# PRBonn/OverlapNet

Measured on AMD Instinct MI355X. Metric: scan-pairs/s (64x900 range images), higher is better.
Workload: dtype f32 (scaled 3-term fp16 split on the fp16 MFMA: 22 significand bits per operand, fp32 accumulate)

## Files before the change

overlapnet_amd/csrc/c3_dense.hip:

```cpp
#include "ovn_internal.h"

typedef _Float16 f16x8 __attribute__((ext_vector_type(8)));
typedef _Float16 f16x4 __attribute__((ext_vector_type(4)));

namespace {

struct ArithF16 {
  typedef _Float16 elem;
  typedef f16x8 v8;
  typedef f16x4 v4;
  static __device__ __forceinline__ f32x4 mfma(v8 a, v8 b, f32x4 c) { return __builtin_amdgcn_mfma_f32_16x16x32_f16(a, b, c, 0, 0, 0); }
};

constexpr int G = OVN_G;
constexpr int OW = OVN_O3_HW;
constexpr int CI = OVN_C2_OUT;
constexpr int CO = OVN_C3_OUT;
constexpr int NBAND = 3;
constexpr int MAX_ROWS = 8;
constexpr int MAX_MT = (MAX_ROWS * OW + 15) / 16;
constexpr int IN_PIX_MAX = (MAX_ROWS + 2) * G;
constexpr int PLANE = IN_PIX_MAX * 8 + 8;
constexpr int NPL = CI / 8;
constexpr size_t LDS_BYTES = 2 * (size_t)NPL * PLANE * sizeof(_Float16) + 64;
constexpr int NW = 8;

__device__ __forceinline__ int band_start(int b) { return b == 0 ? 0 : (b == 1 ? 8 : 15); }
__device__ __forceinline__ int band_rows(int b) { return b == 0 ? 8 : 7; }

constexpr int MT_SPLIT = 6;
template <class A, int NWV, int MSPLIT>
__global__ __launch_bounds__(64 * NWV) void c3_dense_kernel(const float* __restrict__ o2, const typename A::elem* __restrict__ wp,
                                                           const float* __restrict__ b3, const float* __restrict__ wd,
                                                           const unsigned* __restrict__ o2max, float sw3,
                                                           float* __restrict__ partial, float* __restrict__ o3,
                                                           unsigned* __restrict__ arrived, const float* __restrict__ bd,
                                                           float* __restrict__ overlap, float* __restrict__ logit) {
  typedef typename A::elem elem_t;
  typedef typename A::v8 v8_t;
  typedef typename A::v4 v4_t;
  extern __shared__ __attribute__((aligned(16))) unsigned char smem[];
  elem_t* ih = reinterpret_cast<elem_t*>(smem);
  elem_t* il = ih + NPL * PLANE;
  float* red = reinterpret_cast<float*>(il + NPL * PLANE);

  constexpr int HALVES = NW / NWV;
  constexpr int MTW = MSPLIT == 1 ? MAX_MT : MT_SPLIT;
  const int sub = blockIdx.x % (HALVES * MSPLIT);
  const int unit = blockIdx.x / (HALVES * MSPLIT), half = sub % HALVES, mh = sub / HALVES;
  const int mt0 = MT_SPLIT * mh;
  const int pair = unit / NBAND;
  const int band = unit - pair * NBAND;
  const int r0 = band_start(band);
  const int nrows = band_rows(band);
  const int npix = nrows * OW;
  const int nmt = (npix + 15) >> 4;
  const int tid = threadIdx.x;
  const int lane = tid & 63;
  const int wave_l = tid >> 6;
  const int wave = wave_l + NWV * half;
  const int lrow = lane & 15;
  const int g = lane >> 4;

  const elem_t* wsrc = wp + ((size_t)(2 * wave) * 2) * 512 + lane * 8;
  v8_t bq[3][4];
#define C3_LOAD_B(DST, KC)                                                                  \
  {                                                                                         \
    const elem_t* q = wsrc + (size_t)(KC) * (16 * 2 * 512);                                 \
    DST[0] = *reinterpret_cast<const v8_t*>(q);                                           \
    DST[1] = *reinterpret_cast<const v8_t*>(q + 512);                                     \
    DST[2] = *reinterpret_cast<const v8_t*>(q + 1024);                                    \
    DST[3] = *reinterpret_cast<const v8_t*>(q + 1536);                                    \
  }
  C3_LOAD_B(bq[0], 0)
  C3_LOAD_B(bq[1], 1)
  const float s2 = ovn_pow2_scale_for(__uint_as_float(o2max[pair]));
  const float inv = 1.0f / (s2 * sw3);
  {
    const float* src = o2 + ((long long)pair * G + r0) * G * CI;
    const int n4 = (nrows + 2) * G * CI / 4;
    constexpr int PER_THREAD = (MAX_ROWS + 2) * G * CI / 4 / (64 * NWV);
    static_assert(PER_THREAD * 64 * NWV == (MAX_ROWS + 2) * G * CI / 4, "patch does not divide over the threads");
    f32x4 v[PER_THREAD];
#pragma unroll
    for (int k = 0; k < PER_THREAD; ++k) {
      const int i = tid + k * (64 * NWV);
      v[k] = (i < n4) ? *reinterpret_cast<const f32x4*>(src + 4 * i) : (f32x4){0.f, 0.f, 0.f, 0.f};
    }
#pragma unroll
    for (int k = 0; k < PER_THREAD; ++k) {
      const int i = tid + k * (64 * NWV);
      if (i < n4) {
        const int pix = i / (CI / 4);
        const int c = 4 * (i - pix * (CI / 4));
        v4_t h, l;
#pragma unroll
        for (int e = 0; e < 4; ++e) {
          const float x = v[k][e] * s2;
          h[e] = (elem_t)x;
          l[e] = (elem_t)(x - (float)h[e]);
        }
        const int o = (c >> 3) * PLANE + pix * 8 + (c & 7);
        *reinterpret_cast<v4_t*>(ih + o) = h;
        *reinterpret_cast<v4_t*>(il + o) = l;
      }
    }
  }

  int abase[MTW];
#pragma unroll
  for (int mt = 0; mt < MTW; ++mt) {
    int p = 16 * (mt0 + mt) + lrow;
    if (p >= npix) p = npix - 1;
    const int oy = p / OW;
    const int ox = p - oy * OW;
    abase[mt] = g * PLANE + (oy * G + ox) * 8;
  }

  f32x4 acc[MTW][2];
#pragma unroll
  for (int mt = 0; mt < MTW; ++mt) {
    acc[mt][0] = (f32x4){0.f, 0.f, 0.f, 0.f};
    acc[mt][1] = (f32x4){0.f, 0.f, 0.f, 0.f};
  }

#define C3_MFMA2(M0, M1, A0H, A0L, A1H, A1L, SRC)                                                  \
  acc[M0][0] = A::mfma(A0H, SRC[0], acc[M0][0]);          \
  acc[M0][1] = A::mfma(A0H, SRC[2], acc[M0][1]);          \
  acc[M1][0] = A::mfma(A1H, SRC[0], acc[M1][0]);          \
  acc[M1][1] = A::mfma(A1H, SRC[2], acc[M1][1]);          \
  acc[M0][0] = A::mfma(A0L, SRC[0], acc[M0][0]);          \
  acc[M0][1] = A::mfma(A0L, SRC[2], acc[M0][1]);          \
  acc[M1][0] = A::mfma(A1L, SRC[0], acc[M1][0]);          \
  acc[M1][1] = A::mfma(A1L, SRC[2], acc[M1][1]);          \
  acc[M0][0] = A::mfma(A0H, SRC[1], acc[M0][0]);          \
  acc[M0][1] = A::mfma(A0H, SRC[3], acc[M0][1]);          \
  acc[M1][0] = A::mfma(A1H, SRC[1], acc[M1][0]);          \
  acc[M1][1] = A::mfma(A1H, SRC[3], acc[M1][1]);
#define C3_READ_A(BUF, SLOT, MT)                                                            \
  fh[BUF][SLOT] = *reinterpret_cast<const v8_t*>(ih + abase[MT] + toff);                  \
  fl[BUF][SLOT] = *reinterpret_cast<const v8_t*>(il + abase[MT] + toff);
#define C3_STEP(SRC, KC)                                                                    \
  {                                                                                         \
    const int tap = (KC) >> 2;                                                              \
    const int ky = tap / 3;                                                                 \
    const int toff = (ky * G + (tap - 3 * ky)) * 8 + 4 * PLANE * ((KC) & 3);                \
    v8_t fh[2][2], fl[2][2];                                                              \
    C3_READ_A(0, 0, 0)                                                                      \
    C3_READ_A(0, 1, 1)                                                                      \
    _Pragma("unroll") for (int q = 0; q < MTW / 2; ++q) {                                \
      const int cb = q & 1, nb = cb ^ 1;                                                    \
      if (q + 1 < MTW / 2) {                                                             \
        C3_READ_A(nb, 0, 2 * q + 2)                                                         \
        C3_READ_A(nb, 1, 2 * q + 3)                                                         \
      } else if (MTW % 2 == 1 && nmt == MAX_MT) {                                                           \
        C3_READ_A(nb, 0, MTW - 1)                                                        \
      }                                                                                     \
      __builtin_amdgcn_sched_barrier(0);   \
      C3_MFMA2(2 * q, 2 * q + 1, fh[cb][0], fl[cb][0], fh[cb][1], fl[cb][1], SRC)           \
      __builtin_amdgcn_sched_barrier(0);                                                    \
    }                                                                                       \
    if (MTW % 2 == 1 && nmt == MAX_MT) {                               \
      const v8_t ah = fh[(MTW / 2) & 1][0], al = fl[(MTW / 2) & 1][0];              \
      acc[MTW - 1][0] = A::mfma(ah, SRC[0], acc[MTW - 1][0]); \
      acc[MTW - 1][1] = A::mfma(ah, SRC[2], acc[MTW - 1][1]); \
      acc[MTW - 1][0] = A::mfma(al, SRC[0], acc[MTW - 1][0]); \
      acc[MTW - 1][1] = A::mfma(al, SRC[2], acc[MTW - 1][1]); \
      acc[MTW - 1][0] = A::mfma(ah, SRC[1], acc[MTW - 1][0]); \
      acc[MTW - 1][1] = A::mfma(ah, SRC[3], acc[MTW - 1][1]); \
    }                                                                                       \
  }
  __syncthreads();
#pragma unroll 1
  for (int kc = 0; kc < 36; kc += 3) {
    C3_LOAD_B(bq[2], kc + 2)
    C3_STEP(bq[0], kc)
    if (kc + 3 < 36) C3_LOAD_B(bq[0], kc + 3)
    C3_STEP(bq[1], kc + 1)
    if (kc + 4 < 36) C3_LOAD_B(bq[1], kc + 4)
    C3_STEP(bq[2], kc + 2)
  }
#undef C3_LOAD_B
#undef C3_STEP
#undef C3_MFMA2
#undef C3_READ_A

  float s[2] = {0.f, 0.f};
#pragma unroll
  for (int nt = 0; nt < 2; ++nt) {
    const int n = 32 * wave + 16 * nt + lrow;
    const float bv = b3[n];
#pragma unroll
    for (int mt = 0; mt < MTW; ++mt) {
#pragma unroll
      for (int r = 0; r < 4; ++r) {
        const int p = 16 * (mt0 + mt) + 4 * g + r;
        if (p < npix) {
          const float v = fmaxf(fmaf(acc[mt][nt][r], inv, bv), 0.0f);
          const long long fi = (long long)(r0 * OW + p) * CO + n;
          s[(MSPLIT == 1 && mt >= MT_SPLIT) ? 1 : 0] += v * wd[fi];
          if (o3) o3[(long long)pair * OVN_DENSE_IN + fi] = v;
        }
      }
    }
  }
#pragma unroll
  for (int off = 32; off > 0; off >>= 1) {
    s[0] += __shfl_down(s[0], off, 64);
    if (MSPLIT == 1) s[1] += __shfl_down(s[1], off, 64);
  }
  if (lane == 0) {
    red[wave_l] = s[0];
    if (MSPLIT == 1) red[NW + wave_l] = s[1];
  }
  __syncthreads();
  if (tid == 0) {
    float* dst = partial + ((size_t)pair * NBAND + band) * 4;
    if (NWV == NW) {
      dst[0] = (red[0] + red[1]) + (red[2] + red[3]);
      dst[1] = (red[NW + 0] + red[NW + 1]) + (red[NW + 2] + red[NW + 3]);
      dst[2] = (red[4] + red[5]) + (red[6] + red[7]);
      dst[3] = (red[NW + 4] + red[NW + 5]) + (red[NW + 6] + red[NW + 7]);
    } else {
      dst[2 * half + mh] = (red[0] + red[1]) + (red[2] + red[3]);
    }
    if (overlap != nullptr) {
      constexpr unsigned PARTS = NBAND * HALVES * MSPLIT;
      __threadfence();
      const unsigned prev = atomicAdd(arrived + pair, 1u);
      if (prev == PARTS - 1) {
        __threadfence();
        const float* q = partial + (size_t)pair * OVN_DENSE_PARTIALS;
        float z = 0.f;
#pragma unroll
        for (int b = 0; b < NBAND; ++b) {
          const float q0 = __hip_atomic_load(q + 4 * b, __ATOMIC_RELAXED, __HIP_MEMORY_SCOPE_AGENT);
          const float q1 = __hip_atomic_load(q + 4 * b + 1, __ATOMIC_RELAXED, __HIP_MEMORY_SCOPE_AGENT);
          const float q2 = __hip_atomic_load(q + 4 * b + 2, __ATOMIC_RELAXED, __HIP_MEMORY_SCOPE_AGENT);
          const float q3 = __hip_atomic_load(q + 4 * b + 3, __ATOMIC_RELAXED, __HIP_MEMORY_SCOPE_AGENT);
          const float zb = (q0 + q1) + (q2 + q3);
          z = b == 0 ? zb : z + zb;
        }
        z += bd[0];
        if (logit) logit[pair] = z;
        overlap[pair] = 1.0f / (1.0f + expf(-z));
        __hip_atomic_store(arrived + pair, 0u, __ATOMIC_RELAXED, __HIP_MEMORY_SCOPE_AGENT);
      }
    }
  }
}

__global__ __launch_bounds__(256) void dense_finish_kernel(const float* __restrict__ partial, const float* __restrict__ bd, int n,
                                                           float* __restrict__ overlap, float* __restrict__ logit) {
  const int p = blockIdx.x * 256 + threadIdx.x;
  if (p >= n) return;
  const float* q = partial + (size_t)p * OVN_DENSE_PARTIALS;
  float z = 0.f;
#pragma unroll
  for (int b = 0; b < NBAND; ++b) {
    const float zb = (q[4 * b] + q[4 * b + 1]) + (q[4 * b + 2] + q[4 * b + 3]);
    z = b == 0 ? zb : z + zb;
  }
  z += bd[0];
  if (logit) logit[p] = z;
  overlap[p] = 1.0f / (1.0f + expf(-z));
}

}

int ovn_c3_dense_forward(const ovn_ctx* ctx, const float* o2, const unsigned* o2max, int n, float* partial, float* o3,
                         unsigned* arrived, float* overlap, float* logit, hipStream_t stream) {
  OVN_REQUIRE(o2max != nullptr, OVN_ERR_ARG, "ovn_c3_dense_forward: the per-pair maxima of o2 are required");
  OVN_REQUIRE(overlap == nullptr || arrived != nullptr, OVN_ERR_ARG, "ovn_c3_dense_forward: arrival counters missing");
  int rc;
  if (n <= 21) {
    rc = ovn_allow_dynamic_lds(reinterpret_cast<const void*>(c3_dense_kernel<ArithF16, 4, 2>), LDS_BYTES);
    if (rc) return rc;
    hipLaunchKernelGGL((c3_dense_kernel<ArithF16, 4, 2>), dim3(4 * NBAND * n), dim3(64 * 4), LDS_BYTES, stream, o2,
                       reinterpret_cast<const _Float16*>(ctx->c3.wp_h), ctx->c3.bias, ctx->wd, o2max, ctx->c3.sw_h, partial, o3, arrived,
                       ctx->bd, overlap, logit);
  } else {
    rc = ovn_allow_dynamic_lds(reinterpret_cast<const void*>(c3_dense_kernel<ArithF16, NW, 1>), LDS_BYTES);
    if (rc) return rc;
    hipLaunchKernelGGL((c3_dense_kernel<ArithF16, NW, 1>), dim3(NBAND * n), dim3(64 * NW), LDS_BYTES, stream, o2,
                       reinterpret_cast<const _Float16*>(ctx->c3.wp_h), ctx->c3.bias, ctx->wd, o2max, ctx->c3.sw_h, partial, o3,
                       (unsigned*)nullptr, ctx->bd, (float*)nullptr, (float*)nullptr);
    if (overlap != nullptr)
      hipLaunchKernelGGL(dense_finish_kernel, dim3((n + 255) / 256), dim3(256), 0, stream, partial, ctx->bd, n, overlap, logit);
  }
  OVN_HIP_CHECK(hipGetLastError());
  return OVN_OK;
}
```

overlapnet_amd/csrc/ovn_api.hip:

```cpp
#include <stdarg.h>
#include <mutex>
#include <set>
#include <utility>
#include <stdio.h>
#include <stdlib.h>
#include <string.h>

#include <algorithm>
#include "ovn_internal.h"

int ovn_allow_dynamic_lds(const void* kernel, size_t bytes) {
  static std::mutex mu;
  static std::set<std::pair<const void*, int>> done;
  int dev = 0;
  OVN_HIP_CHECK(hipGetDevice(&dev));
  std::lock_guard<std::mutex> lock(mu);
  if (done.count({kernel, dev})) return OVN_OK;
  OVN_HIP_CHECK(hipFuncSetAttribute(kernel, hipFuncAttributeMaxDynamicSharedMemorySize, (int)bytes));
  done.insert({kernel, dev});
  return OVN_OK;
}

static thread_local char g_err[1024] = "";

void ovn_set_error(const char* fmt, ...) {
  va_list ap;
  va_start(ap, fmt);
  vsnprintf(g_err, sizeof(g_err), fmt, ap);
  va_end(ap);
}

int ovn_ws_reserve(ovn_ctx* ctx, size_t bytes, hipStream_t stream) {
  if (bytes <= ctx->ws_bytes) return OVN_OK;
  if (ctx->ws) {
    OVN_HIP_CHECK(hipStreamSynchronize(stream));
    OVN_HIP_CHECK(hipFree(ctx->ws));
    ctx->ws = nullptr;
    ctx->ws_bytes = 0;
    ctx->dbg_o2 = ctx->dbg_o3 = nullptr;
    ctx->dbg_partial = nullptr;
    ctx->dbg_o2max = nullptr;
    ctx->dbg_n = 0;
    ctx->dbg_live = nullptr;
  }
  const size_t want = bytes + bytes / 8;
  OVN_HIP_CHECK(hipMalloc(&ctx->ws, want));
  ctx->ws_bytes = want;
  return OVN_OK;
}

static int ctx_feat_w(const ovn_ctx* ctx) { return ctx->finalized ? ctx->feat_w : OVN_FEAT_W; }

extern "C" {

int ovn_abi_version(void) { return OVN_ABI_VERSION; }

const char* ovn_last_error(void) { return g_err; }

int ovn_create(int device_id, int in_h, int in_w, int in_c, ovn_ctx** out) {
  OVN_REQUIRE(out != nullptr, OVN_ERR_ARG, "ovn_create: out is NULL");
  OVN_REQUIRE(in_h > 0 && in_w > 0 && in_c > 0, OVN_ERR_ARG, "ovn_create: bad input shape %dx%dx%d", in_h, in_w, in_c);
  int ndev = 0;
  OVN_HIP_CHECK(hipGetDeviceCount(&ndev));
  OVN_REQUIRE(device_id >= 0 && device_id < ndev, OVN_ERR_ARG, "ovn_create: device %d not present (%d devices)", device_id, ndev);
  OVN_ON_DEVICE(device_id);
  hipDeviceProp_t prop;
  OVN_HIP_CHECK(hipGetDeviceProperties(&prop, device_id));
  OVN_REQUIRE(strncmp(prop.gcnArchName, "gfx950", 6) == 0, OVN_ERR_STATE,
              "ovn_create: this library is built for gfx950 only, device %d is %s", device_id, prop.gcnArchName);
  ovn_ctx* c = new ovn_ctx();
  c->device = device_id;
  c->in_h = in_h;
  c->in_w = in_w;
  c->in_c = in_c;
  if (const char* e = getenv("OVN_HEAD_CHUNK")) c->head_chunk = atoll(e) > 0 ? atoll(e) : c->head_chunk;
  if (const char* e = getenv("OVN_HEAD_SUBCHUNK")) c->head_sub = atoll(e) >= 0 ? atoll(e) : c->head_sub;
  if (const char* e = getenv("OVN_HEAD_STREAMS")) c->head_streams = atoi(e) == 2 ? 2 : 1;
  if (const char* e = getenv("OVN_YAW_SIDE")) c->head_yaw_side = atoi(e) ? 1 : 0;
  int rc = ovn_spectral_prepare(c, nullptr);
  if (rc) {
    ovn_conv_release(&c->dft);
    if (c->tw64) (void)hipFree(c->tw64);
    delete c;
    return rc;
  }
  *out = c;
  return OVN_OK;
}

int ovn_destroy(ovn_ctx* ctx) {
  if (!ctx) return OVN_OK;
  if (ctx->comm) (void)ovn_comm_destroy(ctx);
  OVN_ON_DEVICE(ctx->device);
  (void)hipDeviceSynchronize();
  for (auto& l : ctx->leg) ovn_conv_release(&l);
  ovn_conv_release(&ctx->c2);
  ovn_conv_release(&ctx->c3);
  ovn_conv_release(&ctx->dft);
  if (ctx->tw64) (void)hipFree(ctx->tw64);
  if (ctx->w1p) (void)hipFree(ctx->w1p);
  if (ctx->b1) (void)hipFree(ctx->b1);
  if (ctx->wd) (void)hipFree(ctx->wd);
  if (ctx->bd) (void)hipFree(ctx->bd);
  if (ctx->w1p_h) (void)hipFree(ctx->w1p_h);
  if (ctx->w2p_h) (void)hipFree(ctx->w2p_h);
  if (ctx->w1raw) (void)hipFree(ctx->w1raw);
  if (ctx->w1sum) (void)hipFree(ctx->w1sum);
  if (ctx->w1col) (void)hipFree(ctx->w1col);
  if (ctx->wsp_h) (void)hipFree(ctx->wsp_h);
  if (ctx->w2sum) (void)hipFree(ctx->w2sum);
  if (ctx->w1p_b3) (void)hipFree(ctx->w1p_b3);
  if (ctx->w2p_b3) (void)hipFree(ctx->w2p_b3);
  if (ctx->w2raw) (void)hipFree(ctx->w2raw);
  if (ctx->ws) (void)hipFree(ctx->ws);
  if (ctx->norm_buf) (void)hipFree(ctx->norm_buf);
  if (ctx->actmax) (void)hipFree(ctx->actmax);
  if (ctx->c3_arrived) (void)hipFree(ctx->c3_arrived);
  if (ctx->seg_dev) (void)hipFree(ctx->seg_dev);
  if (ctx->seg_host) (void)hipHostFree(ctx->seg_host);
  if (ctx->seg_ev) (void)hipEventDestroy(ctx->seg_ev);
  if (ctx->seg_done) (void)hipEventDestroy(ctx->seg_done);
  if (ctx->aux_ready) {
    for (int i = 0; i < 2; ++i) {
      (void)hipStreamDestroy(ctx->aux[i]);
      (void)hipEventDestroy(ctx->ev_join[i]);
    }
    (void)hipEventDestroy(ctx->ev_fork);
  }
  delete ctx;
  return OVN_OK;
}

int ovn_add_leg_layer(ovn_ctx* ctx, const char* name, const float* kernel_dev, const float* bias_dev, int kh, int kw,
                      int cin, int cout, int stride_h, int stride_w, void* stream) {
  OVN_REQUIRE(ctx && name && kernel_dev && bias_dev, OVN_ERR_ARG, "ovn_add_leg_layer: NULL argument");
  OVN_REQUIRE(kh > 0 && kw > 0 && cin > 0 && cout > 0 && stride_h > 0 && stride_w > 0, OVN_ERR_ARG,
              "ovn_add_leg_layer(%s): bad geometry", name);
  OVN_REQUIRE(!ctx->finalized, OVN_ERR_STATE, "ovn_add_leg_layer(%s): context already finalized", name);
  const int expect_cin = ctx->leg.empty() ? ctx->in_c : ctx->leg.back().cout;
  OVN_REQUIRE(cin == expect_cin, OVN_ERR_ARG, "ovn_add_leg_layer(%s): cin=%d but previous layer produces %d", name, cin, expect_cin);
  OVN_ON_DEVICE(ctx->device);
  OvnConvLayer L;
  L.name = name;
  L.kh = kh;
  L.kw = kw;
  L.cin = cin;
  L.cout = cout;
  L.sh = stride_h;
  L.sw = stride_w;
  L.relu = 1;
  int rc = ovn_conv_prepare(&L, kernel_dev, bias_dev, (hipStream_t)stream);
  if (rc) return rc;
  rc = ovn_conv_prepare_f16x3(&L, kernel_dev, (hipStream_t)stream);
  if (rc) {
    ovn_conv_release(&L);
    return rc;
  }
  ctx->leg.push_back(L);
  return OVN_OK;
}

int ovn_set_head_weights(ovn_ctx* ctx, const float* c1k, const float* c1b, const float* c2k, const float* c2b,
                         const float* c3k, const float* c3b, const float* dk, const float* db, void* stream_) {
  OVN_REQUIRE(ctx && c1k && c1b && c2k && c2b && c3k && c3b && dk && db, OVN_ERR_ARG, "ovn_set_head_weights: NULL argument");
  OVN_ON_DEVICE(ctx->device);
  hipStream_t stream = (hipStream_t)stream_;
  {
    ovn_conv_release(&ctx->c2);
    ovn_conv_release(&ctx->c3);
    if (ctx->w1p) (void)hipFree(ctx->w1p);
    if (ctx->b1) (void)hipFree(ctx->b1);
    if (ctx->wd) (void)hipFree(ctx->wd);
    if (ctx->bd) (void)hipFree(ctx->bd);
    if (ctx->w1p_h) (void)hipFree(ctx->w1p_h);
    if (ctx->w2p_h) (void)hipFree(ctx->w2p_h);
    if (ctx->w1raw) (void)hipFree(ctx->w1raw);
    if (ctx->w1sum) (void)hipFree(ctx->w1sum);
    if (ctx->w1col) (void)hipFree(ctx->w1col);
    if (ctx->wsp_h) (void)hipFree(ctx->wsp_h);
      if (ctx->w2sum) (void)hipFree(ctx->w2sum);
    if (ctx->w1p_b3) (void)hipFree(ctx->w1p_b3);
    if (ctx->w2p_b3) (void)hipFree(ctx->w2p_b3);
    if (ctx->w2raw) (void)hipFree(ctx->w2raw);
    ctx->w1p_h = ctx->w2p_h = ctx->wsp_h = ctx->w1p_b3 = ctx->w2p_b3 = nullptr;
    ctx->w1raw = ctx->w1sum = ctx->w1col = ctx->w2sum = ctx->w2raw = nullptr;
    ctx->w1p = ctx->b1 = ctx->wd = ctx->bd = nullptr;
    ctx->head_set = false;
  }
  ctx->head_g = ctx_feat_w(ctx) / ctx->head_s;
  const int hs = ctx->head_s, hg = ctx->head_g;
  OVN_REQUIRE(hg >= 3, OVN_ERR_ARG, "ovn_set_head_weights: conv1size %d leaves %d column groups, c_conv3 needs 3", hs, hg);
  const bool general = (hs != OVN_S);
  int rc = OVN_OK;
  if (!general) {
    rc = ovn_delta_prepare_w1(c1k, &ctx->w1p, stream);
    if (rc) return rc;
  } else {
    const size_t w1_bytes = (size_t)hs * OVN_FEAT_C * OVN_C1_OUT * sizeof(float);
    OVN_HIP_CHECK(hipMalloc((void**)&ctx->w1raw, w1_bytes));
    OVN_HIP_CHECK(hipMemcpyAsync(ctx->w1raw, c1k, w1_bytes, hipMemcpyDeviceToDevice, stream));
  }
  OVN_HIP_CHECK(hipMalloc((void**)&ctx->b1, OVN_C1_OUT * sizeof(float)));
  OVN_HIP_CHECK(hipMemcpyAsync(ctx->b1, c1b, OVN_C1_OUT * sizeof(float), hipMemcpyDeviceToDevice, stream));
  ctx->c2 = OvnConvLayer();
  ctx->c2.name = "c_conv2";
  ctx->c2.kh = hs;
  ctx->c2.kw = 1;
  ctx->c2.cin = OVN_C1_OUT;
  ctx->c2.cout = OVN_C2_OUT;
  ctx->c2.sh = hs;
  ctx->c2.sw = 1;
  ctx->c2.relu = 1;
  rc = ovn_conv_prepare(&ctx->c2, c2k, c2b, stream);
  if (rc) return rc;
  if (!general) {
    rc = ovn_delta_prepare_f16x3(ctx, c1k, c1b, c2k, stream);
    if (rc) return rc;
  }
  ctx->c3 = OvnConvLayer();
  ctx->c3.name = "c_conv3";
  ctx->c3.kh = 3;
  ctx->c3.kw = 3;
  ctx->c3.cin = OVN_C2_OUT;
  ctx->c3.cout = OVN_C3_OUT;
  ctx->c3.sh = 1;
  ctx->c3.sw = 1;
  ctx->c3.relu = 1;
  rc = ovn_conv_prepare(&ctx->c3, c3k, c3b, stream);
  if (rc) return rc;
  if (!general) {
    rc = ovn_conv_prepare_f16x3(&ctx->c3, c3k, stream);
    if (rc) return rc;
  }
  const size_t dense_in = (size_t)(hg - 2) * (hg - 2) * OVN_C3_OUT;
  OVN_HIP_CHECK(hipMalloc((void**)&ctx->wd, dense_in * sizeof(float)));
  OVN_HIP_CHECK(hipMalloc((void**)&ctx->bd, sizeof(float)));
  OVN_HIP_CHECK(hipMemcpyAsync(ctx->wd, dk, dense_in * sizeof(float), hipMemcpyDeviceToDevice, stream));
  OVN_HIP_CHECK(hipMemcpyAsync(ctx->bd, db, sizeof(float), hipMemcpyDeviceToDevice, stream));
  OVN_HIP_CHECK(hipStreamSynchronize(stream));
  ctx->head_set = true;
  return OVN_OK;
}

int ovn_finalize(ovn_ctx* ctx, int* feat_w) {
  OVN_REQUIRE(ctx != nullptr, OVN_ERR_ARG, "ovn_finalize: ctx is NULL");
  OVN_REQUIRE(!ctx->leg.empty(), OVN_ERR_STATE, "ovn_finalize: no leg layers registered");
  int h = ctx->in_h, w = ctx->in_w, c = ctx->in_c;
  for (const auto& l : ctx->leg) {
    OVN_REQUIRE(h >= l.kh && w >= l.kw, OVN_ERR_ARG, "ovn_finalize: layer %s does not fit its %dx%d input", l.name.c_str(), h, w);
    h = (h - l.kh) / l.sh + 1;
    w = (w - l.kw) / l.sw + 1;
    c = l.cout;
  }
  OVN_REQUIRE(h == 1 && w >= OVN_FEAT_W_MIN && w <= OVN_FEAT_W_MAX && c == OVN_FEAT_C, OVN_ERR_ARG,
              "ovn_finalize: leg produces %dx%dx%d, the heads need 1 x W x %d with %d <= W <= %d", h, w, c, OVN_FEAT_C, OVN_FEAT_W_MIN,
              OVN_FEAT_W_MAX);
  OVN_REQUIRE(!ctx->head_set || w / ctx->head_s == ctx->head_g, OVN_ERR_STATE,
              "ovn_finalize: leg width %d gives %d column groups, the head weights were registered for %d", w, w / ctx->head_s,
              ctx->head_g);
  ctx->feat_w = w;
  ctx->finalized = true;
  if (feat_w) *feat_w = w;
  return OVN_OK;
}

int ovn_leg(ovn_ctx* ctx, const float* images_dev, int64_t n, float* features_dev, void* stream_) {
  OVN_REQUIRE(ctx && ctx->finalized, OVN_ERR_STATE, "ovn_leg: context not finalized");
  OVN_REQUIRE(n >= 0, OVN_ERR_ARG, "ovn_leg: n < 0");
  if (n == 0) return OVN_OK;
  OVN_REQUIRE(images_dev && features_dev, OVN_ERR_ARG, "ovn_leg: NULL buffer");
  OVN_ON_DEVICE(ctx->device);
  hipStream_t stream = (hipStream_t)stream_;
  size_t max_act = 0;
  {
    int h = ctx->in_h, w = ctx->in_w;
    for (const auto& l : ctx->leg) {
      h = (h - l.kh) / l.sh + 1;
      w = (w - l.kw) / l.sw + 1;
      const size_t e = (size_t)h * w * l.cout;
      if (e > max_act) max_act = e;
    }
  }
  const int64_t nslices = (n + OVN_LEG_SLICE - 1) / OVN_LEG_SLICE;
  const int64_t slice = (n + nslices - 1) / nslices;
  const size_t buf_bytes = ((size_t)slice * max_act * sizeof(float) + 255) & ~(size_t)255;
  int rc = ovn_ws_reserve(ctx, 2 * buf_bytes, stream);
  if (rc) return rc;
  float* buf[2] = {reinterpret_cast<float*>(ctx->ws), reinterpret_cast<float*>(static_cast<char*>(ctx->ws) + buf_bytes)};
  const size_t in_elems = (size_t)ctx->in_h * ctx->in_w * ctx->in_c;
  const size_t feat_elems = (size_t)ctx->feat_w * OVN_FEAT_C;
  OVN_REQUIRE(ctx->leg.size() + 1 <= OVN_ACTMAX_SLOTS, OVN_ERR_STATE, "ovn_leg: too many leg layers");
  const size_t actmax_bytes = (size_t)OVN_ACTMAX_SLOTS * OVN_LEG_SLICE * OVN_ACTMAX_STRIDE * sizeof(unsigned);
  if (ctx->leg_mode != 0 && !ctx->actmax) OVN_HIP_CHECK(hipMalloc((void**)&ctx->actmax, actmax_bytes));
  for (int64_t s0 = 0; s0 < n; s0 += slice) {
    const int nb = (int)((n - s0 < slice) ? (n - s0) : slice);
    const float* cur = images_dev + (size_t)s0 * in_elems;
    int h = ctx->in_h, w = ctx->in_w;
    if (ctx->leg_mode != 0) {
      OVN_HIP_CHECK(hipMemsetAsync(ctx->actmax, 0, (ctx->leg.size() + 1) * (size_t)slice * OVN_ACTMAX_STRIDE * sizeof(unsigned), stream));
      const bool own = (reinterpret_cast<uintptr_t>(cur) & 15) == 0 && ovn_conv_strip_own_scale(ctx->leg[0], n, h, w);
      if (!own) {
        OvnProfScope ps(ctx, OVN_K_LEG, stream);
        rc = ovn_absmax_forward(cur, nb, (long long)in_elems, ctx->actmax, stream);
        if (rc) return rc;
      }
    }
    for (size_t li = 0; li < ctx->leg.size(); ++li) {
      const bool last = (li + 1 == ctx->leg.size());
      float* dst = last ? features_dev + (size_t)s0 * feat_elems : buf[li & 1];
      int oh = 0, ow = 0;
      if (ctx->leg_mode != 0 && li == 0 && (reinterpret_cast<uintptr_t>(cur) & 15) == 0 && ovn_leg_front_matches(ctx, li, h, w)) {
        OvnProfScope ps(ctx, OVN_K_LEG, stream);
        float* dst2 = buf[(li + 1) & 1];
        rc = ovn_leg_front_forward(ctx, li, cur, nb, h, w, dst2, &oh, &ow, ctx->actmax + (li + 2) * (size_t)slice * OVN_ACTMAX_STRIDE, stream);
        if (rc) return rc;
        cur = dst2;
        h = oh;
        w = ow;
        ++li;
        continue;
      }
// ... 737 lines not shown
```

overlapnet_amd/csrc/ovn_internal.h:

```cpp
#pragma once

#include <hip/hip_runtime.h>
#include <math.h>
#include <stdint.h>

#include <string>
#include <vector>

#include "../../include/ovn_hip.h"

typedef float f32x4 __attribute__((ext_vector_type(4)));

void ovn_set_error(const char* fmt, ...);

#define OVN_HIP_CHECK(expr)                                                                   \
  do {                                                                                        \
    hipError_t _e = (expr);                                                                   \
    if (_e != hipSuccess) {                                                                   \
      ovn_set_error("%s failed: %s (%s:%d)", #expr, hipGetErrorString(_e), __FILE__, __LINE__); \
      return OVN_ERR_HIP;                                                                     \
    }                                                                                         \
  } while (0)

#define OVN_REQUIRE(cond, code, ...)   \
// ... 133 lines not shown
      lo = fminf(lo, L.mn[b][tid]);
      hi = fmaxf(hi, L.mx[b][tid]);
    }
    if (mode == 2) {
      L.m[tid] = (double)lo;
      L.s[tid] = 1.0 / (((double)hi - (double)lo) + 1e-6);
    } else {
      L.m[tid] = (mode == 3) ? sm / (double)W : 0.0;
      L.s[tid] = 0.0;
    }
  }
  __syncthreads();
  if (mode == 2) return;
  const double a = ovn_corr_norm_add(mode);
  for (int t = tid; t < nb * NCH; t += nt) {
    const int c = t % NCH, b = t / NCH;
    const float* p = X + (size_t)(b * OVN_NORM_BLK) * OVN_FEAT_C + c;
    L.part[b][c] = ovn_norm_block_sumsq(p, b < nfull ? OVN_NORM_BLK : tail, L.m[c], a);
  }
  __syncthreads();
  if (tid < NCH) {
    double q = 0.0;
    for (int b = 0; b < nb; ++b) q += L.part[b][tid];
    L.s[tid] = 1.0 / sqrt(q > 1e-12 ? q : 1e-12);
  }
  __syncthreads();
}
#endif

struct OvnHeadScales {
  float sw1 = 1.f, sw2 = 1.f;
  float sws = 1.f;
  float w1_colsum = 0.f;
  float b1_absmax = 0.f;
};

int ovn_allow_dynamic_lds(const void* kernel, size_t bytes);

struct OvnConvLayer {
  std::string name;
  int kh = 0, kw = 0, cin = 0, cout = 0, sh = 1, sw = 1;
  int relu = 1;
  int out_cols = 0;
  int K = 0;
  int nkc = 0;
  float* wp = nullptr;
  float* bias = nullptr;
  void* wp_h = nullptr;
  float sw_h = 1.f;
  void* wp_h16 = nullptr;
};

struct ovn_ctx {
  int device = 0;
  int in_h = 0, in_w = 0, in_c = 0;
  std::vector<OvnConvLayer> leg;
  bool finalized = false;
  int feat_w = 0;
  bool head_set = false;
  int head_s = OVN_S;
  int head_g = OVN_G;
  float* w1p = nullptr;
  float* b1 = nullptr;
  OvnConvLayer c2;
  OvnConvLayer c3;
  void* w1p_h = nullptr;
  void* w2p_h = nullptr;
  float* w1raw = nullptr;
  float* w1sum = nullptr;
  float* w1col = nullptr;
  void* wsp_h = nullptr;
  float* w2sum = nullptr;
  void* w1p_b3 = nullptr;
  void* w2p_b3 = nullptr;
  float* w2raw = nullptr;
  OvnHeadScales hs;
  int leg_mode = 1;
  int head_compact = 1;
  int proj_trig = 0;
  unsigned* actmax = nullptr;
  int head_mode = 1;
  int head_width_split = 0;
  float* wd = nullptr;
  float* bd = nullptr;
  OvnConvLayer dft;
  double* tw64 = nullptr;
  int corr_norm = 0;
  float* norm_buf = nullptr;
  int64_t norm_buf_n = 0;
  void* comm = nullptr;
  int comm_rank = 0, comm_world = 1;
  int64_t head_chunk = 1024;
  int64_t head_sub = 0;
  int head_streams = 1;
  int head_yaw_side = 0;
  bool aux_ready = false;
  hipStream_t aux[2] = {nullptr, nullptr};
  hipEvent_t ev_fork = nullptr, ev_join[2] = {nullptr, nullptr};
  void* ws = nullptr;
  size_t ws_bytes = 0;
  bool prof = false;
  struct ProfRec {
    hipEvent_t a, b;
    int kind;
  };
  std::vector<ProfRec> prof_recs;
  const float* dbg_o2 = nullptr;
  const float* dbg_o3 = nullptr;
  float* dbg_partial = nullptr;
  const unsigned* dbg_o2max = nullptr;
  int64_t dbg_n = 0;
  unsigned* c3_arrived = nullptr;
  int64_t c3_arrived_n = 0;
  const unsigned* dbg_live = nullptr;
  void* seg_host = nullptr;
  void* seg_dev = nullptr;
  size_t seg_cap = 0;
  hipEvent_t seg_ev = nullptr;
  hipEvent_t seg_done = nullptr;
  bool seg_ev_pending = false;
};

enum { OVN_K_LEG = 0, OVN_K_CORR = 1, OVN_K_DELTA = 2, OVN_K_C3 = 3, OVN_K_DENSE = 4, OVN_K_PROJ = 5, OVN_K_SPECTRUM = 6,
       OVN_K_CORR_SPECTRAL = 7, OVN_K_DELTA_PREP = 8, OVN_K_DELTA_C2 = 9, OVN_K_COUNT = 10 };

struct OvnProfScope {
  ovn_ctx* ctx;
  hipStream_t stream;
  hipEvent_t a = nullptr, b = nullptr;
  int kind;
  OvnProfScope(ovn_ctx* c, int k, hipStream_t s) : ctx(c), stream(s), kind(k) {
    if (ctx->prof && hipEventCreate(&a) == hipSuccess && hipEventCreate(&b) == hipSuccess) (void)hipEventRecord(a, stream);
  }
  ~OvnProfScope() {
    if (ctx->prof && a && b) {
      (void)hipEventRecord(b, stream);
      ctx->prof_recs.push_back({a, b, kind});
    }
  }
};

int ovn_ws_reserve(ovn_ctx* ctx, size_t bytes, hipStream_t stream);

int ovn_conv_prepare(OvnConvLayer* L, const float* kernel_dev, const float* bias_dev, hipStream_t stream);
void ovn_conv_release(OvnConvLayer* L);
int ovn_conv_forward(const OvnConvLayer& L, const float* in, int nb, int h, int w, float* out, int* oh,
                     int* ow, hipStream_t stream);

int ovn_conv_prepare_f16x3(OvnConvLayer* L, const float* kernel_dev, hipStream_t stream);
int ovn_conv_forward_f16x3(const OvnConvLayer& L, const float* in, int nb, int h, int w, float* out, int* oh, int* ow,
                           const unsigned* in_max, unsigned* out_max, hipStream_t stream);
int ovn_absmax_forward(const float* x, int n_scans, long long per_scan, unsigned* out_max, hipStream_t stream);

int ovn_delta_prepare_w1(const float* c1_kernel_dev, float** w1p_out, hipStream_t stream);
size_t ovn_delta_pair_bytes(int G);
int ovn_delta_forward(ovn_ctx* ctx, const float* feats_l, const int32_t* lidx, const float* feats_r, const int32_t* ridx, int n,
                      void* scratch, float* overlap, float* logit, hipStream_t stream);
int ovn_dense_sigmoid_forward(const ovn_ctx* ctx, const float* o3, int n, long long dense_in, float* overlap, float* logit,
                              hipStream_t stream);

int ovn_delta_prepare_f16x3(ovn_ctx* ctx, const float* c1_kernel_dev, const float* c1_bias_dev, const float* c2_kernel_dev,
                            hipStream_t stream);
size_t ovn_delta_f16x3_scratch_bytes(int n, bool per_pair_right);
struct OvnSegPass {
  const int32_t* pseg;
  const int32_t* qidx;
  const int64_t* offs;
  int seg0, nseg;
  void* scratch;
};
size_t ovn_delta_f16x3_seg_bytes(int nseg);
int ovn_delta_c12_f16x3_forward(ovn_ctx* ctx, const float* feats_l, const int32_t* lidx, const float* feats_r,
                                const int32_t* ridx, int n, void* scratch, unsigned** o2max_out, float* o2, hipStream_t stream,
                                int pair0 = 0,
                                const float* dcache_l = nullptr,
                                bool a2_done = false,
                                const struct OvnSegPass* seg = nullptr);
float* ovn_delta_f16x3_a2raw(void* scratch, int n);
int ovn_delta_c12_bf16x3_forward(ovn_ctx* ctx, const float* feats_l, const int32_t* lidx, const float* feats_r, const int32_t* ridx,
                                 int n, void* scratch, float* o2, hipStream_t stream, int pair0, bool a2_done);
int ovn_delta_cache_forward(ovn_ctx* ctx, const float* feats, int n, float* cache, hipStream_t stream);
int ovn_delta_walk_stats(ovn_ctx* ctx, int32_t* out16, hipStream_t stream);

size_t ovn_delta_generic_pair_bytes(int W, int G);
int ovn_delta_generic_forward(const ovn_ctx* ctx, const float* feats_l, const int32_t* lidx, const float* feats_r,
                              const int32_t* ridx, int n, void* scratch, float* overlap, float* logit, hipStream_t stream);

size_t ovn_delta_w_split_pair_bytes();
int ovn_delta_w_split_c12_forward(ovn_ctx* ctx, const float* feats_l, const int32_t* lidx, const float* feats_r, const int32_t* ridx,
                                  int n, void* scales, float* o2, hipStream_t stream);

int ovn_corr_forward(const float* feats_l, const int32_t* lidx, const float* feats_r, const int32_t* ridx, int n, int W,
                     int32_t* yaw, float* corr, hipStream_t stream, int norm_mode);

int ovn_spectral_prepare(ovn_ctx* ctx, hipStream_t stream);
int ovn_spectrum_forward(ovn_ctx* ctx, const float* feats, int n, float* spectra, hipStream_t stream);
bool ovn_conv_strip_own_scale(const OvnConvLayer& L, long long call_nb, int h, int w);
int ovn_conv_strip_try(const OvnConvLayer& L, const float* in, int nb, long long call_nb, int h, int w, float* out,
                       const unsigned* in_max, unsigned* out_max, hipStream_t stream);

bool ovn_leg_front_matches(const ovn_ctx* ctx, size_t first, int h, int w);
int ovn_leg_front_forward(const ovn_ctx* ctx, size_t first, const float* in, int nb, int h, int w, float* out, int* oh_out, int* ow_out,
                          unsigned* out_max, hipStream_t stream);

bool ovn_leg_tail_matches(const ovn_ctx* ctx, size_t first, int h, int w);
int ovn_leg_tail_forward(const ovn_ctx* ctx, size_t first, const float* in, int nb, int w, float* out, hipStream_t stream);

int ovn_c3_dense_forward(const ovn_ctx* ctx, const float* o2, const unsigned* o2max, int n, float* partial, float* o3,
                         unsigned* arrived, float* overlap, float* logit, hipStream_t stream);

int ovn_gt_range_forward(const float* points, const int64_t* offsets, int n_scans, long long max_points, const double* ref_poses,
                         const double* inv_cur_pose, int H, int W, double fov_up_deg, double fov_down_deg, double max_range,
                         float* range_out, hipStream_t stream);
int ovn_gt_count_forward(const float* ref_ranges, const float* cur_range, int n, int npix, int32_t* counts, hipStream_t stream);
int ovn_best_match_forward(const float* overlap, const int32_t* yaw, const int32_t* ids, int n, float threshold,
                           int index_offset, int32_t* out, hipStream_t stream);
int ovn_top_k_forward(const float* overlap, const int32_t* yaw, const int32_t* ids, int n, int k, float threshold,
                      int index_offset, int32_t* out, hipStream_t stream);
int ovn_top_k_segments_forward(const float* overlap, const int32_t* yaw, const int32_t* ids, const int64_t* offs_dev, int B, int k,
                               float threshold, int32_t* out, hipStream_t stream);
int ovn_segment_ridx_forward(const int64_t* offs_dev, const int32_t* qidx_dev, int B, int n, int32_t* ridx, int32_t* pseg,
                             hipStream_t stream);
int ovn_corr_spectral_forward(ovn_ctx* ctx, const float* spec_l, const int32_t* lidx, const float* spec_r,
                              const int32_t* ridx, int n, int32_t* yaw, float* corr, hipStream_t stream,
                              const float* a2_feats_r = nullptr, float* a2raw = nullptr);

int ovn_project_forward(ovn_ctx* ctx, const float* points, const int64_t* offsets, int n_scans,
                        int64_t max_points, int H, int W, double fov_up_deg, double fov_down_deg,
                        double max_range, float* range, float* vertex, float* intensity, int32_t* idx,
                        float* normal, float* stacked, int use_depth, int use_normals, int use_intensity,
                        hipStream_t stream);

int ovn_project_semantic_forward(ovn_ctx* ctx, const float* points, const int64_t* offsets, int n_scans, int64_t max_points, int H,
                                 int W, double fov_up_deg, double fov_down_deg, double max_range, const float* probs, int n_classes,
                                 float* range, float* vertex, float* intensity, int32_t* idx, float* normal, float* semantic,
                                 int32_t* sem_idx, float* stacked, int use_depth, int use_normals, int use_semantic, int use_intensity,
                                 hipStream_t stream);
int ovn_projection_angles_forward(const float* points, int64_t n, int H, int W, double fov_up_deg, double fov_down_deg,
                                  double max_range, float* yaw, float* pitch, int32_t* pixel, hipStream_t stream, int trig = 0);
int ovn_normals_forward(const float* range, const float* vertex, int n_scans, int H, int W, float* normal,
                        hipStream_t stream);

int ovn_mfma_selftest(hipStream_t stream);
```

Baseline: 244,400.

## Walk all three bands per block in c3_dense and fuse the dense finish

For large batches each block now handles one scan pair and loops over the three row bands, prefetching the next band's patch and the first B-weight chunks while the current band finishes. The separate dense_finish kernel is removed because the sigmoid is computed in-block. Dense weights are re-laid out once into lane order so each lane reads them as contiguous float4 vectors. The cost is a grid three times smaller with a serial per-block band loop, an extra weight buffer, and more register pressure from the prefetched patch and weights.

New measurement: 245,600, median of 6. About the same (+0.5%).

```diff
diff --git a/overlapnet_amd/csrc/c3_dense.hip b/overlapnet_amd/csrc/c3_dense.hip
--- a/overlapnet_amd/csrc/c3_dense.hip
+++ b/overlapnet_amd/csrc/c3_dense.hip
@@ -29,10 +29,24 @@
 __device__ __forceinline__ int band_rows(int b) { return b == 0 ? 8 : 7; }
 
 constexpr int MT_SPLIT = 6;
-template <class A, int NWV, int MSPLIT>
+constexpr int WDL_ELEMS = NBAND * NW * 2 * MAX_MT * 64 * 4;
+
+template <int PER_THREAD, int NTHR>
+__device__ __forceinline__ void c3_load_patch(f32x4 (&v)[PER_THREAD], const float* __restrict__ o2, int pair, int band, int tid) {
+  const float* src = o2 + ((long long)pair * G + band_start(band)) * G * CI;
+  const int n4 = (band_rows(band) + 2) * G * CI / 4;
+#pragma unroll
+  for (int k = 0; k < PER_THREAD; ++k) {
+    const int i = tid + k * NTHR;
+    v[k] = *reinterpret_cast<const f32x4*>(src + 4 * (i < n4 ? i : tid));
+  }
+}
+
+template <class A, int NWV, int MSPLIT, bool O3>
 __global__ __launch_bounds__(64 * NWV) void c3_dense_kernel(const float* __restrict__ o2, const typename A::elem* __restrict__ wp,
                                                            const float* __restrict__ b3, const float* __restrict__ wd,
-                                                           const unsigned* __restrict__ o2max, float sw3,
+                                                           const float* __restrict__ wdl, const unsigned* __restrict__ o2max,
+                                                           float sw3,
                                                            float* __restrict__ partial, float* __restrict__ o3,
                                                            unsigned* __restrict__ arrived, const float* __restrict__ bd,
                                                            float* __restrict__ overlap, float* __restrict__ logit) {
@@ -45,24 +59,19 @@
   float* red = reinterpret_cast<float*>(il + NPL * PLANE);
 
   constexpr int HALVES = NW / NWV;
+  constexpr bool WALK = NWV == NW;
+  static_assert(!WALK || MSPLIT == 1, "the walking build keeps all m-tiles");
   constexpr int MTW = MSPLIT == 1 ? MAX_MT : MT_SPLIT;
   const int sub = blockIdx.x % (HALVES * MSPLIT);
   const int unit = blockIdx.x / (HALVES * MSPLIT), half = sub % HALVES, mh = sub / HALVES;
   const int mt0 = MT_SPLIT * mh;
-  const int pair = unit / NBAND;
-  const int band = unit - pair * NBAND;
-  const int r0 = band_start(band);
-  const int nrows = band_rows(band);
-  const int npix = nrows * OW;
-  const int nmt = (npix + 15) >> 4;
+  const int pair = WALK ? (int)blockIdx.x : unit / NBAND;
+  int band = WALK ? 0 : unit - pair * NBAND;
   const int tid = threadIdx.x;
-  const int lane = tid & 63;
   const int wave_l = tid >> 6;
   const int wave = wave_l + NWV * half;
-  const int lrow = lane & 15;
-  const int g = lane >> 4;
-
-  const elem_t* wsrc = wp + ((size_t)(2 * wave) * 2) * 512 + lane * 8;
+
+  const elem_t* wsrc = wp + ((size_t)(2 * wave) * 2) * 512 + (tid & 63) * 8;
   v8_t bq[3][4];
 #define C3_LOAD_B(DST, KC)                                                                  \
   {                                                                                         \
@@ -74,22 +83,27 @@
   }
   C3_LOAD_B(bq[0], 0)
   C3_LOAD_B(bq[1], 1)
+  constexpr int PER_THREAD = (MAX_ROWS + 2) * G * CI / 4 / (64 * NWV);
+  static_assert(PER_THREAD * 64 * NWV == (MAX_ROWS + 2) * G * CI / 4, "patch does not divide over the threads");
+  f32x4 v[PER_THREAD];
+  c3_load_patch<PER_THREAD, 64 * NWV>(v, o2, pair, band, tid);
+  float z = 0.f;
+
+  for (;;) {
+  int tidu = tid;
+  if (WALK) asm volatile("" : "+v"(tidu));
+  const int lane = tidu & 63, lrow = lane & 15, g = lane >> 4;
+  const int r0 = band_start(band);
+  const int nrows = band_rows(band);
+  const int npix = nrows * OW;
+  const int nmt = (npix + 15) >> 4;
   const float s2 = ovn_pow2_scale_for(__uint_as_float(o2max[pair]));
   const float inv = 1.0f / (s2 * sw3);
   {
-    const float* src = o2 + ((long long)pair * G + r0) * G * CI;
     const int n4 = (nrows + 2) * G * CI / 4;
-    constexpr int PER_THREAD = (MAX_ROWS + 2) * G * CI / 4 / (64 * NWV);
-    static_assert(PER_THREAD * 64 * NWV == (MAX_ROWS + 2) * G * CI / 4, "patch does not divide over the threads");
-    f32x4 v[PER_THREAD];
 #pragma unroll
     for (int k = 0; k < PER_THREAD; ++k) {
-      const int i = tid + k * (64 * NWV);
-      v[k] = (i < n4) ? *reinterpret_cast<const f32x4*>(src + 4 * i) : (f32x4){0.f, 0.f, 0.f, 0.f};
-    }
-#pragma unroll
-    for (int k = 0; k < PER_THREAD; ++k) {
-      const int i = tid + k * (64 * NWV);
+      const int i = tidu + k * (64 * NWV);
       if (i < n4) {
         const int pix = i / (CI / 4);
         const int c = 4 * (i - pix * (CI / 4));
@@ -175,118 +189,170 @@
   for (int kc = 0; kc < 36; kc += 3) {
     C3_LOAD_B(bq[2], kc + 2)
     C3_STEP(bq[0], kc)
-    if (kc + 3 < 36) C3_LOAD_B(bq[0], kc + 3)
+    if (kc + 3 < 36) C3_LOAD_B(bq[0], kc + 3) else if (WALK) C3_LOAD_B(bq[0], 0)
     C3_STEP(bq[1], kc + 1)
-    if (kc + 4 < 36) C3_LOAD_B(bq[1], kc + 4)
+    if (kc + 4 < 36) C3_LOAD_B(bq[1], kc + 4) else if (WALK) C3_LOAD_B(bq[1], 1)
     C3_STEP(bq[2], kc + 2)
+  }
+
+  float s[2] = {0.f, 0.f};
+  const float bv2[2] = {b3[32 * wave + lrow], b3[32 * wave + 16 + lrow]};
+  __builtin_amdgcn_sched_barrier(0);
+  f32x4 w4[2][MTW];
+  if constexpr (WALK) {
+    const float* wl = wdl + ((size_t)(band * NW + wave) * 2 * MAX_MT * 64 + lane) * 4;
+#pragma unroll
+    for (int nt = 0; nt < 2; ++nt)
+#pragma unroll
+      for (int mt = 0; mt < MTW; ++mt) w4[nt][mt] = *reinterpret_cast<const f32x4*>(wl + (nt * MAX_MT + mt) * 256);
+  }
+  __builtin_amdgcn_sched_barrier(0);
+#pragma unroll
+  for (int nt = 0; nt < 2; ++nt) {
+    const int nch = 32 * wave + 16 * nt + lrow;
+    const float bv = bv2[nt];
+#pragma unroll
+    for (int mt = 0; mt < MTW; ++mt) {
+#pragma unroll
+      for (int r = 0; r < 4; ++r) {
+        const int p = 16 * (mt0 + mt) + 4 * g + r;
+        const float a = fmaxf(fmaf(acc[mt][nt][r], inv, bv), 0.0f);
+        float& sum = s[(MSPLIT == 1 && mt >= MT_SPLIT) ? 1 : 0];
+        if constexpr (WALK) {
+          const float t = fmaf(a, w4[nt][mt][r], sum);
+          sum = p < npix ? t : sum;
+        } else if (p < npix) {
+          sum = fmaf(a, wd[(long long)(r0 * OW + p) * CO + nch], sum);
+        }
+      }
+    }
+  }
+  if (WALK ? O3 : o3 != nullptr) {
+#pragma unroll
+    for (int nt = 0; nt < 2; ++nt) {
+      const int nch = 32 * wave + 16 * nt + lrow;
+      const float bv = b3[nch];
+#pragma unroll
+      for (int mt = 0; mt < MTW; ++mt) {
+#pragma unroll
+        for (int r = 0; r < 4; ++r) {
+          const int p = 16 * (mt0 + mt) + 4 * g + r;
+          if (p < npix) o3[(long long)pair * OVN_DENSE_IN + (long long)(r0 * OW + p) * CO + nch] = fmaxf(fmaf(acc[mt][nt][r], inv, bv), 0.0f);
+        }
+      }
+    }
+  }
+#pragma unroll
+  for (int off = 32; off > 0; off >>= 1) {
+    s[0] += __shfl_down(s[0], off, 64);
+    if (MSPLIT == 1) s[1] += __shfl_down(s[1], off, 64);
+  }
+  if (lane == 0) {
+    red[wave_l] = s[0];
+    if (MSPLIT == 1) red[NW + wave_l] = s[1];
+  }
+  __syncthreads();
+  if (tid == 0) {
+    float* dst = partial ? partial + ((size_t)pair * NBAND + band) * 4 : nullptr;
+    if constexpr (WALK) {
+      const float q0 = (red[0] + red[1]) + (red[2] + red[3]);
+      const float q1 = (red[NW + 0] + red[NW + 1]) + (red[NW + 2] + red[NW + 3]);
+      const float q2 = (red[4] + red[5]) + (red[6] + red[7]);
+      const float q3 = (red[NW + 4] + red[NW + 5]) + (red[NW + 6] + red[NW + 7]);
+      if (dst) {
+        dst[0] = q0;
+        dst[1] = q1;
+        dst[2] = q2;
+        dst[3] = q3;
+      }
+      const float zb = (q0 + q1) + (q2 + q3);
+      z = band == 0 ? zb : z + zb;
+      if (band == NBAND - 1 && overlap != nullptr) {
+        z += bd[0];
+        if (logit) logit[pair] = z;
+        overlap[pair] = 1.0f / (1.0f + expf(-z));
+      }
+    } else {
+      dst[2 * half + mh] = (red[0] + red[1]) + (red[2] + red[3]);
+      if (overlap != nullptr) {
+        constexpr unsigned PARTS = NBAND * HALVES * MSPLIT;
+        __threadfence();
+        const unsigned prev = atomicAdd(arrived + pair, 1u);
+        if (prev == PARTS - 1) {
+          __threadfence();
+          const float* q = partial + (size_t)pair * OVN_DENSE_PARTIALS;
+          float zz = 0.f;
+#pragma unroll
+          for (int b = 0; b < NBAND; ++b) {
+            const float q0 = __hip_atomic_load(q + 4 * b, __ATOMIC_RELAXED, __HIP_MEMORY_SCOPE_AGENT);
+            const float q1 = __hip_atomic_load(q + 4 * b + 1, __ATOMIC_RELAXED, __HIP_MEMORY_SCOPE_AGENT);
+            const float q2 = __hip_atomic_load(q + 4 * b + 2, __ATOMIC_RELAXED, __HIP_MEMORY_SCOPE_AGENT);
+            const float q3 = __hip_atomic_load(q + 4 * b + 3, __ATOMIC_RELAXED, __HIP_MEMORY_SCOPE_AGENT);
+            const float zb = (q0 + q1) + (q2 + q3);
+            zz = b == 0 ? zb : zz + zb;
+          }
+          zz += bd[0];
+          if (logit) logit[pair] = zz;
+          overlap[pair] = 1.0f / (1.0f + expf(-zz));
+          __hip_atomic_store(arrived + pair, 0u, __ATOMIC_RELAXED, __HIP_MEMORY_SCOPE_AGENT);
+        }
+      }
+    }
+  }
+  if (!WALK || band == NBAND - 1) break;
+  ++band;
+  c3_load_patch<PER_THREAD, 64 * NWV>(v, o2, pair, band, tidu);
   }
 #undef C3_LOAD_B
 #undef C3_STEP
 #undef C3_MFMA2
 #undef C3_READ_A
-
-  float s[2] = {0.f, 0.f};
-#pragma unroll
-  for (int nt = 0; nt < 2; ++nt) {
-    const int n = 32 * wave + 16 * nt + lrow;
-    const float bv = b3[n];
-#pragma unroll
-    for (int mt = 0; mt < MTW; ++mt) {
-#pragma unroll
-      for (int r = 0; r < 4; ++r) {
-        const int p = 16 * (mt0 + mt) + 4 * g + r;
-        if (p < npix) {
-          const float v = fmaxf(fmaf(acc[mt][nt][r], inv, bv), 0.0f);
-          const long long fi = (long long)(r0 * OW + p) * CO + n;
-          s[(MSPLIT == 1 && mt >= MT_SPLIT) ? 1 : 0] += v * wd[fi];
-          if (o3) o3[(long long)pair * OVN_DENSE_IN + fi] = v;
-        }
-      }
-    }
-  }
-#pragma unroll
-  for (int off = 32; off > 0; off >>= 1) {
-    s[0] += __shfl_down(s[0], off, 64);
-    if (MSPLIT == 1) s[1] += __shfl_down(s[1], off, 64);
-  }
-  if (lane == 0) {
-    red[wave_l] = s[0];
-    if (MSPLIT == 1) red[NW + wave_l] = s[1];
-  }
-  __syncthreads();
-  if (tid == 0) {
-    float* dst = partial + ((size_t)pair * NBAND + band) * 4;
-    if (NWV == NW) {
-      dst[0] = (red[0] + red[1]) + (red[2] + red[3]);
-      dst[1] = (red[NW + 0] + red[NW + 1]) + (red[NW + 2] + red[NW + 3]);
-      dst[2] = (red[4] + red[5]) + (red[6] + red[7]);
-      dst[3] = (red[NW + 4] + red[NW + 5]) + (red[NW + 6] + red[NW + 7]);
-    } else {
-      dst[2 * half + mh] = (red[0] + red[1]) + (red[2] + red[3]);
-    }
-    if (overlap != nullptr) {
-      constexpr unsigned PARTS = NBAND * HALVES * MSPLIT;
-      __threadfence();
-      const unsigned prev = atomicAdd(arrived + pair, 1u);
-      if (prev == PARTS - 1) {
-        __threadfence();
-        const float* q = partial + (size_t)pair * OVN_DENSE_PARTIALS;
-        float z = 0.f;
-#pragma unroll
-        for (int b = 0; b < NBAND; ++b) {
-          const float q0 = __hip_atomic_load(q + 4 * b, __ATOMIC_RELAXED, __HIP_MEMORY_SCOPE_AGENT);
-          const float q1 = __hip_atomic_load(q + 4 * b + 1, __ATOMIC_RELAXED, __HIP_MEMORY_SCOPE_AGENT);
-          const float q2 = __hip_atomic_load(q + 4 * b + 2, __ATOMIC_RELAXED, __HIP_MEMORY_SCOPE_AGENT);
-          const float q3 = __hip_atomic_load(q + 4 * b + 3, __ATOMIC_RELAXED, __HIP_MEMORY_SCOPE_AGENT);
-          const float zb = (q0 + q1) + (q2 + q3);
-          z = b == 0 ? zb : z + zb;
-        }
-        z += bd[0];
-        if (logit) logit[pair] = z;
-        overlap[pair] = 1.0f / (1.0f + expf(-z));
-        __hip_atomic_store(arrived + pair, 0u, __ATOMIC_RELAXED, __HIP_MEMORY_SCOPE_AGENT);
-      }
-    }
-  }
-}
-
-__global__ __launch_bounds__(256) void dense_finish_kernel(const float* __restrict__ partial, const float* __restrict__ bd, int n,
-                                                           float* __restrict__ overlap, float* __restrict__ logit) {
-  const int p = blockIdx.x * 256 + threadIdx.x;
-  if (p >= n) return;
-  const float* q = partial + (size_t)p * OVN_DENSE_PARTIALS;
-  float z = 0.f;
-#pragma unroll
-  for (int b = 0; b < NBAND; ++b) {
-    const float zb = (q[4 * b] + q[4 * b + 1]) + (q[4 * b + 2] + q[4 * b + 3]);
-    z = b == 0 ? zb : z + zb;
-  }
-  z += bd[0];
-  if (logit) logit[p] = z;
-  overlap[p] = 1.0f / (1.0f + expf(-z));
-}
-
+}
+
+__global__ __launch_bounds__(256) void dense_lane_order_kernel(const float* __restrict__ wd, float* __restrict__ wdl) {
+  const int i = blockIdx.x * 256 + threadIdx.x;
+  if (i >= WDL_ELEMS) return;
+  const int r = i & 3, lane = (i >> 2) & 63;
+  int rest = i >> 8;
+  const int mt = rest % MAX_MT;
+  rest /= MAX_MT;
+  const int nt = rest & 1;
+  rest >>= 1;
+  const int wave = rest % NW, band = rest / NW;
+  const int p = 16 * mt + 4 * (lane >> 4) + r;
+  const int nch = 32 * wave + 16 * nt + (lane & 15);
+  wdl[i] = p < band_rows(band) * OW ? wd[(size_t)(band_start(band) * OW + p) * CO + nch] : 0.0f;
+}
+
+}
+
+int ovn_c3_dense_prepare(ovn_ctx* ctx, hipStream_t stream) {
+  OVN_REQUIRE(ctx->wd != nullptr && ctx->wd_lane == nullptr, OVN_ERR_STATE, "ovn_c3_dense_prepare: Dense weights not registered");
+  OVN_HIP_CHECK(hipMalloc((void**)&ctx->wd_lane, (size_t)WDL_ELEMS * sizeof(float)));
+  hipLaunchKernelGGL(dense_lane_order_kernel, dim3((WDL_ELEMS + 255) / 256), dim3(256), 0, stream, ctx->wd, ctx->wd_lane);
+  OVN_HIP_CHECK(hipGetLastError());
+  return OVN_OK;
 }
 
 int ovn_c3_dense_forward(const ovn_ctx* ctx, const float* o2, const unsigned* o2max, int n, float* partial, float* o3,
                          unsigned* arrived, float* overlap, float* logit, hipStream_t stream) {
   OVN_REQUIRE(o2max != nullptr, OVN_ERR_ARG, "ovn_c3_dense_forward: the per-pair maxima of o2 are required");
-  OVN_REQUIRE(overlap == nullptr || arrived != nullptr, OVN_ERR_ARG, "ovn_c3_dense_forward: arrival counters missing");
   int rc;
   if (n <= 21) {
-    rc = ovn_allow_dynamic_lds(reinterpret_cast<const void*>(c3_dense_kernel<ArithF16, 4, 2>), LDS_BYTES);
+    OVN_REQUIRE(overlap == nullptr || arrived != nullptr, OVN_ERR_ARG, "ovn_c3_dense_forward: arrival counters missing");
+    rc = ovn_allow_dynamic_lds(reinterpret_cast<const void*>(c3_dense_kernel<ArithF16, 4, 2, false>), LDS_BYTES);
     if (rc) return rc;
-    hipLaunchKernelGGL((c3_dense_kernel<ArithF16, 4, 2>), dim3(4 * NBAND * n), dim3(64 * 4), LDS_BYTES, stream, o2,
-                       reinterpret_cast<const _Float16*>(ctx->c3.wp_h), ctx->c3.bias, ctx->wd, o2max, ctx->c3.sw_h, partial, o3, arrived,
-                       ctx->bd, overlap, logit);
+    hipLaunchKernelGGL((c3_dense_kernel<ArithF16, 4, 2, false>), dim3(4 * NBAND * n), dim3(64 * 4), LDS_BYTES, stream, o2,
+                       reinterpret_cast<const _Float16*>(ctx->c3.wp_h), ctx->c3.bias, ctx->wd, ctx->wd_lane, o2max, ctx->c3.sw_h,
+                       partial, o3, arrived, ctx->bd, overlap, logit);
   } else {
-    rc = ovn_allow_dynamic_lds(reinterpret_cast<const void*>(c3_dense_kernel<ArithF16, NW, 1>), LDS_BYTES);
+    OVN_REQUIRE(ctx->wd_lane != nullptr, OVN_ERR_STATE, "ovn_c3_dense_forward: the lane-order Dense weights are missing");
+    auto kern = o3 ? c3_dense_kernel<ArithF16, NW, 1, true> : c3_dense_kernel<ArithF16, NW, 1, false>;
+    rc = ovn_allow_dynamic_lds(reinterpret_cast<const void*>(kern), LDS_BYTES);
     if (rc) return rc;
-    hipLaunchKernelGGL((c3_dense_kernel<ArithF16, NW, 1>), dim3(NBAND * n), dim3(64 * NW), LDS_BYTES, stream, o2,
-                       reinterpret_cast<const _Float16*>(ctx->c3.wp_h), ctx->c3.bias, ctx->wd, o2max, ctx->c3.sw_h, partial, o3,
-                       (unsigned*)nullptr, ctx->bd, (float*)nullptr, (float*)nullptr);
-    if (overlap != nullptr)
-      hipLaunchKernelGGL(dense_finish_kernel, dim3((n + 255) / 256), dim3(256), 0, stream, partial, ctx->bd, n, overlap, logit);
+    hipLaunchKernelGGL(kern, dim3(n), dim3(64 * NW), LDS_BYTES, stream, o2, reinterpret_cast<const _Float16*>(ctx->c3.wp_h),
+                       ctx->c3.bias, ctx->wd, ctx->wd_lane, o2max, ctx->c3.sw_h, partial, o3, (unsigned*)nullptr, ctx->bd, overlap,
+                       logit);
   }
   OVN_HIP_CHECK(hipGetLastError());
   return OVN_OK;
diff --git a/overlapnet_amd/csrc/ovn_api.hip b/overlapnet_amd/csrc/ovn_api.hip
--- a/overlapnet_amd/csrc/ovn_api.hip
+++ b/overlapnet_amd/csrc/ovn_api.hip
@@ -101,6 +101,7 @@
   if (ctx->w1p) (void)hipFree(ctx->w1p);
   if (ctx->b1) (void)hipFree(ctx->b1);
   if (ctx->wd) (void)hipFree(ctx->wd);
+  if (ctx->wd_lane) (void)hipFree(ctx->wd_lane);
   if (ctx->bd) (void)hipFree(ctx->bd);
   if (ctx->w1p_h) (void)hipFree(ctx->w1p_h);
   if (ctx->w2p_h) (void)hipFree(ctx->w2p_h);
@@ -171,6 +172,7 @@
     if (ctx->w1p) (void)hipFree(ctx->w1p);
     if (ctx->b1) (void)hipFree(ctx->b1);
     if (ctx->wd) (void)hipFree(ctx->wd);
+    if (ctx->wd_lane) (void)hipFree(ctx->wd_lane);
     if (ctx->bd) (void)hipFree(ctx->bd);
     if (ctx->w1p_h) (void)hipFree(ctx->w1p_h);
     if (ctx->w2p_h) (void)hipFree(ctx->w2p_h);
@@ -184,7 +186,7 @@
     if (ctx->w2raw) (void)hipFree(ctx->w2raw);
     ctx->w1p_h = ctx->w2p_h = ctx->wsp_h = ctx->w1p_b3 = ctx->w2p_b3 = nullptr;
     ctx->w1raw = ctx->w1sum = ctx->w1col = ctx->w2sum = ctx->w2raw = nullptr;
-    ctx->w1p = ctx->b1 = ctx->wd = ctx->bd = nullptr;
+    ctx->w1p = ctx->b1 = ctx->wd = ctx->wd_lane = ctx->bd = nullptr;
     ctx->head_set = false;
   }
   ctx->head_g = ctx_feat_w(ctx) / ctx->head_s;
@@ -237,6 +239,10 @@
   OVN_HIP_CHECK(hipMalloc((void**)&ctx->bd, sizeof(float)));
   OVN_HIP_CHECK(hipMemcpyAsync(ctx->wd, dk, dense_in * sizeof(float), hipMemcpyDeviceToDevice, stream));
   OVN_HIP_CHECK(hipMemcpyAsync(ctx->bd, db, sizeof(float), hipMemcpyDeviceToDevice, stream));
+  if (!general && hg == OVN_G) {
+    rc = ovn_c3_dense_prepare(ctx, stream);
+    if (rc) return rc;
+  }
   OVN_HIP_CHECK(hipStreamSynchronize(stream));
   ctx->head_set = true;
   return OVN_OK;
diff --git a/overlapnet_amd/csrc/ovn_internal.h b/overlapnet_amd/csrc/ovn_internal.h
--- a/overlapnet_amd/csrc/ovn_internal.h
+++ b/overlapnet_amd/csrc/ovn_internal.h
@@ -239,6 +239,7 @@
   int head_mode = 1;
   int head_width_split = 0;
   float* wd = nullptr;
+  float* wd_lane = nullptr;
   float* bd = nullptr;
   OvnConvLayer dft;
   double* tw64 = nullptr;
@@ -365,6 +366,7 @@
 
 int ovn_c3_dense_forward(const ovn_ctx* ctx, const float* o2, const unsigned* o2max, int n, float* partial, float* o3,
                          unsigned* arrived, float* overlap, float* logit, hipStream_t stream);
+int ovn_c3_dense_prepare(ovn_ctx* ctx, hipStream_t stream);
 
 int ovn_gt_range_forward(const float* points, const int64_t* offsets, int n_scans, long long max_points, const double* ref_poses,
                          const double* inv_cur_pose, int H, int W, double fov_up_deg, double fov_down_deg, double max_range,
```
